# AlgoLab/rs-vgaligner

Measured on AMD Instinct MI355X. Metric: aligned reads/sec (10 kbp ONT vs HLA graph), higher is better.
Workload: dtype int32+f64

## Files before the change

### include/vga_hip.h

```cpp
#ifndef VGA_HIP_H
#define VGA_HIP_H

#include <stddef.h>
#include <stdint.h>

#ifdef __cplusplus
extern "C" {
#endif

#define VGA_OK 0
#define VGA_ERR_ARG (-1)
#define VGA_ERR_HIP (-2)
#define VGA_ERR_NOMEM (-3)
#define VGA_ERR_UNSUPPORTED (-4)
#define VGA_ERR_NO_INDEX (-5)
#define VGA_ERR_NO_DEVICE (-6)
#define VGA_ERR_POOL (-7)

#define VGA_NO_PRED (-1)

#define VGA_MAX_KMER_LENGTH 32

typedef struct vga_ctx vga_ctx;

// ... 45 lines not shown
    uint64_t max_gap;
    uint32_t chain_min_n_anchors;
    int only_forward;
    int emit_dp;
    int32_t strands;
} vga_map_params;
#define VGA_STRANDS_FORWARD 0
#define VGA_STRANDS_BOTH 1
void vga_map_default_params(vga_map_params *p);

typedef struct {
    uint64_t n_reads;
    uint64_t n_anchors;
    uint64_t *anchor_off;
    uint32_t *anchor_id;
    uint32_t *query_begin;
    uint32_t *target_begin;
    uint32_t *target_end;
    double *max_chain_score;
    int32_t *best_pred_id;
    double *curr_max;
    uint64_t n_chains;
    uint64_t *chain_off;
    uint8_t *chain_placeholder;
    uint64_t *chain_anchor_off;
    uint32_t *chain_anchor_idx;
    float ms_probe, ms_sort, ms_chain, ms_total;
    uint64_t n_hits;
    uint8_t *strand;
} vga_map_result;

int vga_map_batch(vga_batch *b, const vga_map_params *params, vga_map_result **out);
void vga_map_result_free(vga_map_result *r);

typedef struct {
    uint64_t n_chains;
    uint64_t *text_off;
    char *text;
    float ms_total;
} vga_chain_text;
int vga_chain_paths_text(vga_ctx *ctx, const vga_map_result *chains, vga_chain_text **out);
void vga_chain_text_free(vga_chain_text *t);

typedef struct {
    int32_t match;
    int32_t mismatch;
    int32_t gap_open1;
    int32_t gap_ext1;
    int32_t gap_open2;
    int32_t gap_ext2;
    int32_t wb;
    int32_t remain_rule;
    double wf;
} vga_poa_params;
#define VGA_REMAIN_LONGEST_PATH 0
#define VGA_REMAIN_FIRST_OUT_EDGE 1
void vga_poa_default_params(vga_poa_params *p);

typedef struct {
    uint64_t n;
    uint8_t *ok;
    int32_t *best_score;
    uint64_t *path_off;
    uint32_t *abpoa_nodes;
    uint32_t *graph_nodes;
    uint32_t *aln_start_offset;
// ... 152 lines not shown
```

### rs-vgaligner_amd/binding.py

```python
from __future__ import annotations

import ctypes as C
import os
from typing import List, Optional, Sequence

import numpy as np

_HERE = os.path.dirname(os.path.abspath(__file__))
LIB_PATH = os.environ.get("VGA_LIB") or os.path.join(_HERE, "libvga_hip.so")

VGA_OK = 0
VGA_MAX_KMER_LENGTH = 32
VGA_STRANDS_FORWARD = 0
VGA_STRANDS_BOTH = 1
ERR_NAMES = {-1: "VGA_ERR_ARG", -2: "VGA_ERR_HIP", -3: "VGA_ERR_NOMEM", -4: "VGA_ERR_UNSUPPORTED",
             -5: "VGA_ERR_NO_INDEX", -6: "VGA_ERR_NO_DEVICE", -7: "VGA_ERR_POOL"}

PILEUP_COLUMNS = ("A", "C", "G", "T", "N", "del", "ins")

ABI_SYMBOLS = [
    "vga_ctx_create", "vga_ctx_destroy", "vga_last_error", "vga_ctx_synchronize", "vga_abi_version",
    "vga_index_upload", "vga_batch_create", "vga_batch_destroy", "vga_batch_strands", "vga_map_default_params", "vga_map_batch",
    "vga_map_result_free", "vga_poa_default_params", "vga_poa_result_free", "vga_poa_batch", "vga_align_batch",
    "vga_align_result_free", "vga_last_kernel_times", "vga_chain_paths_text", "vga_chain_text_free",
    "vga_align_prepare", "vga_ctx_set_pool_fraction", "vga_ctx_set_host_threads",
    "vga_index_build_kmers", "vga_index_kmers_free",
    "vga_coverage_begin", "vga_coverage_read", "vga_coverage_reset", "vga_coverage_end",
    "vga_path_support_begin", "vga_path_support_read", "vga_path_support_last", "vga_path_support_reset", "vga_path_support_end",
    "vga_path_support_lists",
    "vga_pileup_begin", "vga_pileup_read", "vga_pileup_reset", "vga_pileup_end",
    "vga_genotype_begin", "vga_genotype_read", "vga_genotype_reset", "vga_genotype_end", "vga_genotype_pairs",
    "vga_genotype_lik_table", "vga_genotype_lik_begin", "vga_genotype_lik_read", "vga_genotype_lik_reset", "vga_genotype_lik_end",
    "vga_genotype_lik_pairs", "vga_genotype_lik_source",
    "vga_path_edit_begin", "vga_path_edit_read", "vga_path_edit_last", "vga_path_edit_reset", "vga_path_edit_end", "vga_path_edit_pairs",
    "vga_variant_call", "vga_variant_call_table",
    "vga_insertion_begin", "vga_insertion_read", "vga_insertion_reset", "vga_insertion_end", "vga_insertion_call", "vga_insertion_call_table",
    "vga_phase_begin", "vga_phase_read", "vga_phase_reset", "vga_phase_end", "vga_phase_links", "vga_phase_links_lists", "vga_phase_chain",
    "vga_phase_tags", "vga_phase_tags_lists",
    "vga_haplotype_counts", "vga_haplotype_counts_lists", "vga_haplotype_jobs", "vga_haplotype_call",
]

GENOTYPE_TILE = 64
GENOTYPE_READS = 32
GENOTYPE_MIN_CHUNKS = 4
GENOTYPE_MAX_PATHS = 4096

GENOTYPE_LIK_TILE = 128
GENOTYPE_LIK_READS = 32
GENOTYPE_LIK_MIN_CHUNKS = 4
GENOTYPE_LIK_MAX_GROUP_READS = 2048
GENOTYPE_LIK_MAX_PATHS = 4096
GENOTYPE_LIK_MAX_LAMBDA = 4096
GENOTYPE_LIK_MAX_CAP = 255
GENOTYPE_LIK_LAMBDA = 512
GENOTYPE_LIK_CAP = 64
VGA_GL_FROM_SUPPORT = 0
# ... 108 lines not shown


class KernelTime(C.Structure):
    _fields_ = [("name", C.c_char_p), ("ms", C.c_float), ("launches", C.c_uint32), ("algorithmic_bytes", C.c_uint64),
                ("busy_ms", C.c_float), ("reserved", C.c_uint32)]


_lib = None


def load_library():
    global _lib
    if _lib is not None:
        return _lib
    if not os.path.exists(LIB_PATH):
        raise RuntimeError(f"{LIB_PATH} is missing: build it with `python -c 'import __graft_entry__ as g; g.build()'` "
                           "(there is no CPU fallback)")
    L = C.CDLL(LIB_PATH)
    vp = C.c_void_p
    L.vga_ctx_create.argtypes = [C.c_int, _P(vp)]
    L.vga_ctx_destroy.argtypes = [vp]
    L.vga_last_error.argtypes = [vp]
    L.vga_last_error.restype = C.c_char_p
    L.vga_ctx_synchronize.argtypes = [vp]
    L.vga_index_upload.argtypes = [vp, _P(IndexDesc)]
    L.vga_batch_create.argtypes = [vp, C.c_char_p, _P(C.c_uint64), C.c_uint64, _P(vp)]
    L.vga_batch_destroy.argtypes = [vp]
    if hasattr(L, "vga_batch_strands"):
        L.vga_batch_strands.argtypes = [vp, C.c_int, _P(C.c_char), _P(C.c_char)]
        L.vga_batch_strands.restype = C.c_int
    L.vga_map_default_params.argtypes = [_P(MapParams)]
    L.vga_map_batch.argtypes = [vp, _P(MapParams), _P(_P(MapResult))]
    L.vga_map_result_free.argtypes = [_P(MapResult)]
    L.vga_poa_default_params.argtypes = [_P(PoaParams)]
    L.vga_poa_result_free.argtypes = [_P(PoaResult)]
    L.vga_poa_batch.argtypes = [vp, C.c_uint64, _P(C.c_uint64), _P(C.c_uint64), C.c_char_p, _P(C.c_uint64),
                                _P(C.c_uint32), _P(C.c_uint32), _P(C.c_uint64), C.c_char_p, _P(PoaParams),
                                _P(_P(PoaResult))]
    L.vga_align_batch.argtypes = [vp, _P(MapResult), C.c_uint32, _P(PoaParams), _P(_P(AlignResult))]
    L.vga_align_result_free.argtypes = [_P(AlignResult)]
    L.vga_last_kernel_times.argtypes = [vp, _P(KernelTime), C.c_int]
    L.vga_chain_paths_text.argtypes = [vp, _P(MapResult), _P(_P(ChainText))]
    L.vga_align_prepare.argtypes = [vp, C.c_uint64, C.c_uint32]
    L.vga_align_prepare.restype = C.c_int
    L.vga_ctx_set_pool_fraction.argtypes = [vp, C.c_double]
    L.vga_ctx_set_pool_fraction.restype = C.c_int
    L.vga_ctx_set_host_threads.argtypes = [vp, C.c_uint32]
    L.vga_ctx_set_host_threads.restype = C.c_int
    L.vga_chain_text_free.argtypes = [_P(ChainText)]
    L.vga_index_build_kmers.argtypes = [vp, _P(IndexDesc), C.c_uint64, C.c_uint64]
    L.vga_index_build_kmers.restype = C.c_int
    L.vga_index_kmers_free.argtypes = [_P(IndexDesc)]
    L.vga_index_kmers_free.restype = None
    if hasattr(L, "vga_coverage_begin"):
        for name in ("vga_coverage_begin", "vga_coverage_reset", "vga_coverage_end"):
            getattr(L, name).argtypes = [vp]
            getattr(L, name).restype = C.c_int
        L.vga_coverage_read.argtypes = [vp, _P(C.c_uint32), _P(C.c_uint32), _P(C.c_uint32), _P(C.c_uint64)]
        L.vga_coverage_read.restype = C.c_int
    if hasattr(L, "vga_path_support_begin"):
        u64p, u32p = _P(C.c_uint64), _P(C.c_uint32)
        L.vga_path_support_begin.argtypes = [vp, C.c_uint32, u64p, u64p, u64p]
        L.vga_path_support_read.argtypes = [vp, u64p, u64p, u64p, u64p, u64p, u64p]
        L.vga_path_support_last.argtypes = [vp, C.c_uint64, u32p, u32p]
        L.vga_path_support_reset.argtypes = [vp]
        L.vga_path_support_end.argtypes = [vp]
# ... 311 lines not shown
        self.poa_value_cells = int(r.poa_value_cells)
        self.ms = {"subgraph": r.ms_subgraph, "dp": r.ms_dp, "traceback": r.ms_traceback, "total": r.ms_total}
        L.vga_align_result_free(ptr)


class Batch:
    def __init__(self, ctx: "Context", seqs: Sequence):
        self.ctx = ctx
        L = ctx.L
        self.seqs = list(seqs)
        raw = [s if isinstance(s, (bytes, bytearray)) else s.encode() for s in self.seqs]
        self._concat = b"".join(raw)
        off = np.zeros(len(self.seqs) + 1, dtype=np.uint64)
        if self.seqs:
            off[1:] = np.cumsum([len(s) for s in raw], dtype=np.uint64)
        self._off = off
        h = C.c_void_p()
        ctx._check(L.vga_batch_create(ctx.h, self._concat, _u64p(off), len(self.seqs), C.byref(h)))
        self.h = h

    def strands(self, from_host: bool = False):
        n = len(self._concat)
        fwd, rev = C.create_string_buffer(max(1, n)), C.create_string_buffer(max(1, n))
        self.ctx._check(self.ctx.L.vga_batch_strands(self.h, 1 if from_host else 0, fwd, rev))
        return fwd.raw[:n], rev.raw[:n]

    def map(self, params: Optional[MapParams] = None) -> MapOut:
        L = self.ctx.L
        p = params or default_map_params()
        out = _P(MapResult)()
        self.ctx._check(L.vga_map_batch(self.h, C.byref(p), C.byref(out)))
        return MapOut(L, out)

    def align(self, chains: MapOut, best_n: int = 1, params: Optional[PoaParams] = None) -> AlignOut:
        L = self.ctx.L
        p = params or default_poa_params()
        out = _P(AlignResult)()
        self.ctx._check(L.vga_align_batch(self.h, chains._ptr, best_n, C.byref(p), C.byref(out)))
        self.ctx._last_reads = len(self.seqs)
        return AlignOut(L, out)

    def map_raw(self, map_params: Optional[MapParams] = None, on_results=None) -> dict:
        L = self.ctx.L
        mp = map_params
        if mp is None:
            mp = default_map_params()
            mp.emit_dp = 0
        m = _P(MapResult)()
        self.ctx._check(L.vga_map_batch(self.h, C.byref(mp), C.byref(m)))
        try:
            q = m.contents
            if on_results is not None:
                on_results(q, None)
            R = int(q.n_reads)
            ph = np.ctypeslib.as_array(q.chain_placeholder, shape=(int(q.n_chains),)) if int(q.n_chains) else np.zeros(0, np.uint8)
            co = np.ctypeslib.as_array(q.chain_off, shape=(R + 1,)) if R else np.zeros(1, np.uint64)
            mapped = int((ph[co[:-1].astype(np.int64)] == 0).sum()) if R else 0
            return dict(n_reads=R, aligned=mapped, n_anchors=int(q.n_anchors), n_hits=int(q.n_hits), n_chains=int(q.n_chains),
                        ms_map=float(q.ms_total), ms_probe=float(q.ms_probe), ms_sort=float(q.ms_sort), ms_chain=float(q.ms_chain),
                        kernels=self.ctx.kernel_times())
        finally:
            L.vga_map_result_free(m)

    def map_align_raw(self, map_params: Optional[MapParams] = None, best_n: int = 1,
                      poa_params: Optional[PoaParams] = None, on_results=None) -> dict:
        import time as _t
# ... 533 lines not shown
```

### rs-vgaligner_amd/csrc/vga_align.hip

```cpp
#include "vga_align_plan.hpp"
#include "vga_common.hpp"
#include "vga_coverage.hpp"
#include "vga_path_edit.hpp"
#include "vga_path_support.hpp"
#include "vga_pileup.hpp"
#include "vga_insertion.hpp"
#include "vga_poa_internal.hpp"
#include "vga_subgraph_host.hpp"

#include <algorithm>
#include <atomic>
#include <chrono>
#include <memory>

extern "C" void vga_align_result_free(vga_align_result *r)
{
    if (!r) return;
    free(r->aligned); free(r->path_off); free(r->path_handles); free(r->path_length); free(r->path_start);
    free(r->path_end); free(r->block_length); free(r->best_score); free(r->cigar_off); free(r->cigar);
    free(r->cs_off); free(r->cs);
    free(r);
}

namespace {
// ... 48 lines not shown
    int device_store_rest();
    void host_walk();
    int run_poa();
    int begin_result();
    void pick_winners();
    int count_winners();
    int fill_result();
};

int align_call::reverse_complements()
{
    bool any_rev = false;
    if (m->strand)
        for (uint64_t r = 0; r < R && !any_rev; r++) any_rev = m->strand[r] != 0;
    if (!any_rev) return VGA_OK;
    const int rc = vga_batch_revcomp_device(b);
    if (rc != VGA_OK) return rc;
    vga_batch_revcomp_host(b);
    tr.mark("reverse complement");
    return VGA_OK;
}

int align_call::plan()
{
    const char *refused = on_device ? nullptr : cov ? "read coverage is not counted" : ps ? "path support is not scored" : pu ? "the pileup is not counted" : ia ? "the inserted letters are not counted" : nullptr;
    if (refused)
        return vga_set_error(ctx, VGA_ERR_UNSUPPORTED, "vga_align_batch: %s under VGA_SUBGRAPH=host (the subgraph handles are then on the host only)", refused);
    align_select(m, align_best_n, prob_read, prob_chain, read_prob0);
    n = prob_read.size();
    proxy.resize(n);
    west.resize(n);
    descs.resize(n);
    std::atomic<int> has_reverse{0};
    vga_parallel_for(n, [&](uint64_t p) {
        const align_prob a = align_plan_problem(m, prob_read[p], prob_chain[p], qlen(prob_read[p]), ctx->index.k, sw);
        proxy[p] = a.proxy; west[p] = a.west; descs[p] = a.desc;
        if (a.reverse) has_reverse = 1;
    });
    std::vector<uint32_t> ord(n);
    std::iota(ord.begin(), ord.end(), 0u);
    if (on_device) {
        ord = align_launch_order(proxy);
        align_permute(prob_read, ord); align_permute(prob_chain, ord); align_permute(proxy, ord); align_permute(west, ord); align_permute(descs, ord);
    }
    slot_of = align_slot_of(ord);
    if (has_reverse)
        return vga_set_error(ctx, VGA_ERR_UNSUPPORTED,
                             "a chain to be aligned holds reverse-strand anchors: RangeOrient::Reverse / Both (src/align.rs:365-387) is not supported");
    feed.views.resize(n);
    q_src.resize(on_device ? n : 0);
    for (uint64_t p = 0; p < n; p++) {
        const uint64_t r = prob_read[p];
        feed.views[p] = {nullptr, nullptr, 0, nullptr, nullptr, 0, b->reads.data() + q_off(r), qlen(r)};
        if (on_device) q_src[p] = q_off(r);
    }
    feed.proxy = proxy.data();
    return VGA_OK;
}

int align_call::device_store()
{
    vga_timers_reset(ctx);
    feed.keep_timers = true;
    auto ta = std::chrono::steady_clock::now();
    double mean_west = 0;
    const uint64_t split = align_store_split(west, sw, &mean_west);
    if (sw.trace)
        fprintf(stderr, "[vga-trace] align: mean width term of the launch-order proxy %.0f: the subgraph store is built in %s\n", mean_west,
                split == n ? "one part" : "two parts");
    const int rc = sg_prepare(ctx, descs.data(), q_src.data(), prob_read.data(), n, split, b->d_reads, params->remain_rule, store);
    if (rc != VGA_OK) return rc;
// ... 229 lines not shown
```

### rs-vgaligner_amd/csrc/vga_align_plan.hpp

```cpp
#pragma once

#include <algorithm>
#include <cmath>
#include <cstdint>
#include <cstdlib>
#include <cstring>
#include <numeric>
#include <vector>

#include "../../include/vga_hip.h"
#include "vga_sg_records.hpp"

struct align_switches {
    bool sg_host = false;
    uint32_t giant_rows = 24000u;
    double giant_cells = 1.5e8;
    bool has_sg_split = false;
    long sg_split = 0;
    bool trace = false;
};

static inline align_switches align_read_switches()
{
    align_switches s;
    if (const char *e = getenv("VGA_SUBGRAPH")) s.sg_host = strstr(e, "host") != nullptr;
    if (const char *e = getenv("VGA_GIANT_ROWS")) s.giant_rows = (uint32_t)atol(e);
    if (const char *e = getenv("VGA_GIANT_CELLS")) s.giant_cells = atof(e);
    if (const char *e = getenv("VGA_SG_SPLIT")) { s.has_sg_split = true; s.sg_split = atol(e); }
    if (const char *e = getenv("VGA_TRACE")) s.trace = atoi(e) != 0;
    return s;
}

static inline void align_select(const vga_map_result *m, uint32_t best_n, std::vector<uint64_t> &prob_read, std::vector<uint64_t> &prob_chain,
                                std::vector<uint64_t> &read_prob0)
{
    const uint64_t R = m->n_reads;
    prob_read.clear();
    prob_chain.clear();
    read_prob0.assign(R + 1, 0);
    for (uint64_t r = 0; r < R; r++) {
        read_prob0[r] = prob_read.size();
        const uint64_t c0 = m->chain_off[r], c1 = m->chain_off[r + 1];
        const uint64_t take = std::min<uint64_t>(best_n, c1 - c0);
        for (uint64_t c = c0; c < c0 + take; c++)
            if (!m->chain_placeholder[c]) { prob_read.push_back(r); prob_chain.push_back(c); }
    }
    read_prob0[R] = prob_read.size();
}

struct align_prob {
    sg_desc desc;
    uint32_t lo, hi;
    float west;
    double proxy;
    bool reverse;
};

static inline align_prob align_plan_problem(const vga_map_result *m, uint64_t r, uint64_t c, uint32_t qlen, uint32_t k, const align_switches &sw)
{
    align_prob o = {};
    const uint64_t a0 = m->anchor_off[r];
    const uint64_t c0 = m->chain_anchor_off[c], c1 = m->chain_anchor_off[c + 1];
    uint32_t lo = 0xFFFFFFFFu, hi = 0, pmin = 0xFFFFFFFFu, pmax = 0;
    for (uint64_t t = c0; t < c1; t++) {
        const uint64_t ai = a0 + m->chain_anchor_idx[t];
        lo = std::min(lo, m->target_begin[ai]);
        hi = std::max(hi, m->target_end[ai]);
        if ((m->target_begin[ai] | m->target_end[ai]) >> 31) o.reverse = true;
        const uint32_t s = m->target_begin[ai], e = m->target_end[ai] - 1;
        pmin = std::min(pmin, std::min(s, e));
        pmax = std::max(pmax, std::max(s, e));
    }
    o.lo = lo;
    o.hi = hi;
    const double q_first = c1 > c0 ? (double)m->query_begin[a0 + m->chain_anchor_idx[c0]] : 0.0;
    const double q_last = c1 > c0 ? (double)m->query_begin[a0 + m->chain_anchor_idx[c1 - 1]] + (double)k : (double)qlen;
    const double uncovered = q_first + std::max(0.0, (double)qlen - q_last);
    const double rows = (double)(hi > lo ? hi - lo : 0) + 1.6 * uncovered;
    o.west = (float)(650.0 + 0.3 * std::max(0.0, 0.85 * rows - (double)qlen));
    o.proxy = rows * (double)o.west;
    if (rows >= 0.85 * (double)sw.giant_rows) o.proxy += 1e13;
    if (c1 > c0) {
        const uint64_t fa = a0 + m->chain_anchor_idx[c0], la = a0 + m->chain_anchor_idx[c1 - 1];
        o.desc = {pmin, pmax, m->query_begin[fa], m->target_begin[fa], m->query_begin[la], m->target_end[la], qlen, 0u};
    }
    return o;
}

static inline std::vector<uint32_t> align_launch_order(const std::vector<double> &proxy)
{
    std::vector<uint32_t> ord(proxy.size());
    std::iota(ord.begin(), ord.end(), 0u);
    std::stable_sort(ord.begin(), ord.end(), [&](uint32_t x, uint32_t y) { return proxy[x] > proxy[y]; });
    return ord;
}

static inline std::vector<uint32_t> align_slot_of(const std::vector<uint32_t> &ord)
{
    std::vector<uint32_t> slot_of(ord.size());
    for (size_t i = 0; i < ord.size(); i++) slot_of[ord[i]] = (uint32_t)i;
    return slot_of;
}

template <typename T>
static inline void align_permute(std::vector<T> &v, const std::vector<uint32_t> &ord)
{
    std::vector<T> w(v.size());
    for (size_t i = 0; i < ord.size(); i++) w[i] = v[ord[i]];
    v.swap(w);
}

static inline uint64_t align_store_split(const std::vector<float> &west, const align_switches &sw, double *mean_west = nullptr)
{
    const uint64_t n = west.size();
    uint64_t split = n > 3072 ? 2048 : n;
    double wsum = 0;
    for (uint64_t i = 0; i < n; i++) wsum += west[i];
    if (n && wsum / (double)n <= 900.0) split = n;
    if (mean_west) *mean_west = n ? wsum / (double)n : 0.0;
// ... 13 lines not shown
```

### rs-vgaligner_amd/csrc/vga_common.hpp

```cpp
#pragma once

#include <hip/hip_runtime.h>
#include <sys/mman.h>

#include <chrono>
#include <cstdarg>
#include <cstdint>
#include <cstdio>
#include <cstdlib>
#include <cstring>
#include <atomic>
#include <memory>
#include <mutex>
#include <new>
#include <string>
#include <thread>
#include <vector>

#include "../../include/vga_hip.h"
#include "vga_probe_hash.hpp"

#define VGA_ABI_VERSION 6

template <typename T>
// ... 64 lines not shown
    std::vector<hipEvent_t> event_pool;
    size_t events_used = 0;
    struct agg_t {
        std::string name;
        float ms;
        uint32_t launches;
        uint64_t bytes;
        float busy_ms;
    };
    std::vector<agg_t> last_times;
    int n_cu = 256;
    vga_owned<void> map_ws{nullptr, nullptr};
    vga_owned<struct poa_ws> poa_ws{nullptr, nullptr};
    vga_owned<void> sg_ws{nullptr, nullptr};
    vga_owned<void> gaf_ws{nullptr, nullptr};
    std::vector<struct vga_batch *> batches;
};

struct vga_batch {
    vga_ctx *ctx = nullptr;
    int device = 0;
    uint64_t n_reads = 0;
    uint64_t total_bases = 0;
    std::vector<uint64_t> read_off;
    std::vector<char> reads;
    char *d_reads = nullptr;
    uint64_t *d_read_off = nullptr;
    bool rc_dev = false, rc_host = false;
    uint64_t *d_read_off2 = nullptr;
};
int vga_batch_revcomp_device(vga_batch *b);
void vga_batch_revcomp_host(vga_batch *b);

int vga_set_error(vga_ctx *ctx, int code, const char *fmt, ...);
void vga_index_release(vga_dev_index &ix);
int vga_index_load_graph(vga_ctx *ctx, const vga_index_desc *d);

#define VGA_HIP_CHECK(ctx, call)                                                               \
    do {                                                                                       \
        hipError_t e_ = (call);                                                                \
        if (e_ != hipSuccess)                                                                  \
            return vga_set_error((ctx), VGA_ERR_HIP, "%s failed: %s (%s:%d)", #call,           \
                                 hipGetErrorString(e_), __FILE__, __LINE__);                   \
    } while (0)
#define VGA_HIP_CHECK_OOM(ctx, call)                                                         \
    do {                                                                                       \
        hipError_t e_ = (call);                                                                \
        if (e_ != hipSuccess)                                                                  \
            return vga_set_error((ctx), e_ == hipErrorOutOfMemory ? VGA_ERR_NOMEM : VGA_ERR_HIP, \
                                 "%s failed: %s (%s:%d)", #call, hipGetErrorString(e_), __FILE__, __LINE__); \
    } while (0)

template <typename T>
T *xmalloc(size_t n)
{
    return (T *)malloc((n ? n : 1) * sizeof(T));
}

template <typename T, void (*FREE)(T *)>
struct vga_result_guard {
    T *p = nullptr;
    const hipStream_t *wait[2] = {nullptr, nullptr};
    vga_result_guard() = default;
    vga_result_guard(const vga_result_guard &) = delete;
    vga_result_guard &operator=(const vga_result_guard &) = delete;
    ~vga_result_guard()
// ... 132 lines not shown
```

### rs-vgaligner_amd/csrc/vga_map.hip

```cpp
#include "vga_common.hpp"

#include <algorithm>
#include <chrono>
#include <cmath>
#include <memory>

#define VGA_WAVE 64
#define VGA_PROBE_NT 256
#define VGA_SORT_NT 256
#define VGA_NONE32 0xFFFFFFFFu

__device__ __forceinline__ uint32_t vga_lane() { return threadIdx.x & 63u; }

__device__ __forceinline__ uint32_t vga_wave_incl_scan(uint32_t v)
{
    uint32_t lane = vga_lane();
#pragma unroll
    for (int d = 1; d < 64; d <<= 1) {
        uint32_t o = __shfl_up(v, d, 64);
        if (lane >= (uint32_t)d) v += o;
    }
    return v;
}

__device__ __forceinline__ uint32_t vga_block_excl_scan_256(uint32_t v, uint32_t *ws, uint32_t &total)
{
    uint32_t incl = vga_wave_incl_scan(v);
    uint32_t w = threadIdx.x >> 6;
    if (vga_lane() == 63) ws[w] = incl;
    __syncthreads();
    uint32_t w0 = ws[0], w1 = ws[1], w2 = ws[2], w3 = ws[3];
    uint32_t before = (w > 0 ? w0 : 0) + (w > 1 ? w1 : 0) + (w > 2 ? w2 : 0);
    total = w0 + w1 + w2 + w3;
    __syncthreads();
    return before + incl - v;
}

__device__ __forceinline__ uint32_t vga_base_code_dev(uint8_t c)
// ... 351 lines not shown
            int pnext;
            while ((pnext = vpred[cur]) >= 0) {
                if (lane == 0) { vpred[cur] = -1; buf[wpos] = (uint32_t)cur; }
                __threadfence_block();
                wpos++;
                len++;
                cur = pnext;
            }
            if (lane == 0) buf[wpos] = (uint32_t)cur;
            wpos++;
            len++;
            if (len >= min_anchors) {
                if (lane == 0) buf[hdr] = len;
                nch++;
            } else {
                wpos = hdr;
            }
        }
    }
    if (lane == 0) { chain_cnt[r] = nch; chain_words[r] = wpos; }
}

__global__ __launch_bounds__(256) void k_chain_compact(const uint64_t *__restrict__ anchor_off, const uint32_t *__restrict__ chain_words,
                                                       const uint64_t *__restrict__ woff, const uint32_t *__restrict__ chain_buf,
                                                       uint32_t *__restrict__ comp)
{
    const uint64_t r = blockIdx.x;
    const uint32_t *src = chain_buf + 3 * anchor_off[r] + 2 * r;
    uint32_t *dst = comp + woff[r];
    const uint32_t n = chain_words[r];
    for (uint32_t i = threadIdx.x; i < n; i += blockDim.x) dst[i] = src[i];
}

__global__ __launch_bounds__(256) void k_strand_pick(uint32_t R, const uint64_t *__restrict__ anchor_off, const double *__restrict__ curr_max,
                                                     const uint32_t *__restrict__ chain_cnt, const uint32_t *__restrict__ chain_words,
                                                     uint8_t *__restrict__ strand, uint32_t *__restrict__ sel, uint32_t *__restrict__ sel_anchors,
                                                     double *__restrict__ sel_curr_max, uint32_t *__restrict__ sel_chain_cnt,
                                                     uint32_t *__restrict__ sel_chain_words)
{
    const uint32_t r = blockIdx.x * 256 + threadIdx.x;
    if (r >= R) return;
    const uint32_t rv = R + r;
    const bool rev = chain_cnt[rv] > 0 && (chain_cnt[r] == 0 || curr_max[rv] > curr_max[r]);
    const uint32_t s = rev ? rv : r;
    strand[r] = rev ? 1 : 0;
    sel[r] = s;
    sel_anchors[r] = (uint32_t)(anchor_off[s + 1] - anchor_off[s]);
    sel_curr_max[r] = curr_max[s];
    sel_chain_cnt[r] = chain_cnt[s];
    sel_chain_words[r] = chain_words[s];
}

__global__ __launch_bounds__(256) void k_strand_scan(uint32_t R, const uint32_t *__restrict__ cnt, uint64_t *__restrict__ off)
{
    __shared__ uint32_t ws[4];
    uint64_t carry = 0;
    for (uint32_t c0 = 0; c0 < R; c0 += 256) {
        const uint32_t i = c0 + threadIdx.x;
        const uint32_t v = i < R ? cnt[i] : 0u;
        uint32_t total;
        const uint32_t ex = vga_block_excl_scan_256(v, ws, total);
        if (i < R) off[i] = carry + ex;
        carry += total;
    }
    if (threadIdx.x == 0) off[R] = carry;
}
// ... 23 lines not shown
}

__global__ __launch_bounds__(256) void k_chain_compact_sel(const uint32_t *__restrict__ sel, const uint64_t *__restrict__ anchor_off,
                                                           const uint32_t *__restrict__ sel_chain_words, const uint64_t *__restrict__ woff,
                                                           const uint32_t *__restrict__ chain_buf, uint32_t *__restrict__ comp)
{
    const uint64_t r = blockIdx.x, s = sel[r];
    const uint32_t *src = chain_buf + 3 * anchor_off[s] + 2 * s;
    uint32_t *dst = comp + woff[r];
    const uint32_t n = sel_chain_words[r];
    for (uint32_t i = threadIdx.x; i < n; i += blockDim.x) dst[i] = src[i];
}

namespace {

struct map_ws {
    vga_dbuf<uint32_t> cnt;
    vga_dbuf<uint64_t> anchor_off;
    vga_dbuf<uint32_t> a_qb, a_tb, a_te, a_idx, key_b, val_b, s_qb, s_tb, s_te;
    vga_dbuf<double> f, curr_max, gap_cost;
    vga_dbuf<int32_t> pred_id, pred_pos;
    vga_dbuf<uint32_t> chain_buf, chain_cnt, chain_words, key_a, chain_comp;
    vga_dbuf<uint64_t> chain_woff;
    vga_dbuf<uint8_t> strand;
    vga_dbuf<uint32_t> sel, sel_anchors, sel_chain_cnt, sel_chain_words, g_qb, g_tb, g_te, g_id;
    vga_dbuf<uint64_t> sel_off;
    vga_dbuf<double> sel_curr_max, g_f;
    vga_dbuf<int32_t> g_pred;
    vga_hbuf<uint64_t> h_chain_woff;
    vga_hbuf<uint32_t> h_chain_cnt, h_chain_words, h_cnt;
    vga_hbuf<double> h_curr_max;
    hipStream_t st_copy = nullptr;
    hipEvent_t ev_sorted = nullptr;
    ~map_ws()
    {
        if (st_copy) (void)hipStreamDestroy(st_copy);
        if (ev_sorted) (void)hipEventDestroy(ev_sorted);
    }
};

}

extern "C" void vga_map_result_free(vga_map_result *r)
{
    if (!r) return;
    free(r->anchor_off);
    free(r->anchor_id);
    free(r->query_begin);
    free(r->target_begin);
    free(r->target_end);
    free(r->max_chain_score);
    free(r->best_pred_id);
    free(r->curr_max);
    free(r->chain_off);
    free(r->chain_placeholder);
    free(r->chain_anchor_off);
    free(r->chain_anchor_idx);
    free(r->strand);
    free(r);
}

namespace {

struct map_source {
    const double *curr_max = nullptr;
    const uint32_t *chain_cnt = nullptr, *chain_words = nullptr;
    const uint32_t *ids = nullptr;
    const double *f = nullptr;
    const int32_t *pred = nullptr;
};

struct map_call {
    vga_ctx *const ctx;
    vga_batch *const b;
    const vga_map_params *const params;
    const vga_dev_index &ix;
    const uint64_t R;
    const bool all_orients;
// ... 252 lines not shown
    VGA_HIP_CHECK(ctx, hipMemcpyAsync(ws.h_curr_max.p, src.curr_max, R * 8, hipMemcpyDeviceToHost, st));
    VGA_HIP_CHECK(ctx, hipMemcpyAsync(ws.h_chain_cnt.p, src.chain_cnt, R * 4, hipMemcpyDeviceToHost, st));
    VGA_HIP_CHECK(ctx, hipMemcpyAsync(ws.h_chain_words.p, src.chain_words, R * 4, hipMemcpyDeviceToHost, st));
    VGA_HIP_CHECK(ctx, hipStreamSynchronize(st));
    return VGA_OK;
}

int map_call::gather_picked()
{
    const size_t As = (size_t)res->anchor_off[R];
    res->n_anchors = As;
    if (!alloc_anchor_arrays(As)) return nomem();
    VGA_HIP_CHECK(ctx, ws.g_qb.reserve(As)); VGA_HIP_CHECK(ctx, ws.g_tb.reserve(As)); VGA_HIP_CHECK(ctx, ws.g_te.reserve(As));
    if (emit_dp) { VGA_HIP_CHECK(ctx, ws.g_id.reserve(As)); VGA_HIP_CHECK(ctx, ws.g_f.reserve(As)); VGA_HIP_CHECK(ctx, ws.g_pred.reserve(As)); }
    const int tg = vga_timer_begin(ctx, "strand_gather", (uint64_t)As * 2 * (12 + (emit_dp ? 16 : 0)) + R * 20);
    hipLaunchKernelGGL(k_strand_gather, dim3((unsigned)R), dim3(256), 0, st, ws.sel.p, ws.anchor_off.p, ws.sel_off.p, ws.s_qb.p, ws.s_tb.p,
                       ws.s_te.p, perm, ws.f.p, ws.pred_id.p, ws.g_qb.p, ws.g_tb.p, ws.g_te.p, emit_dp ? ws.g_id.p : nullptr,
                       emit_dp ? ws.g_f.p : nullptr, emit_dp ? ws.g_pred.p : nullptr);
    vga_timer_end(ctx, tg);
    if (As) {
        VGA_HIP_CHECK(ctx, hipMemcpyAsync(res->query_begin, ws.g_qb.p, As * 4, hipMemcpyDeviceToHost, st));
        VGA_HIP_CHECK(ctx, hipMemcpyAsync(res->target_begin, ws.g_tb.p, As * 4, hipMemcpyDeviceToHost, st));
        VGA_HIP_CHECK(ctx, hipMemcpyAsync(res->target_end, ws.g_te.p, As * 4, hipMemcpyDeviceToHost, st));
    }
    src.ids = ws.g_id.p;
    src.f = ws.g_f.p;
    src.pred = ws.g_pred.p;
    return VGA_OK;
}

int map_call::fetch_chains()
{
    const size_t An_res = (size_t)res->n_anchors;
    for (uint64_t r = 0; r < R; r++) { ws.h_chain_woff.p[r] = chain_total_words; chain_total_words += ws.h_chain_words.p[r]; }
    ws.h_chain_woff.p[R] = chain_total_words;
    chain_words_host.reset(xmalloc<uint32_t>(chain_total_words + 2));
    if (!chain_words_host) return nomem();
    if (chain_total_words) {
        VGA_HIP_CHECK(ctx, ws.chain_comp.reserve(chain_total_words + 2));
        VGA_HIP_CHECK(ctx, hipMemcpyAsync(ws.chain_woff.p, ws.h_chain_woff.p, (R + 1) * 8, hipMemcpyHostToDevice, st));
        if (both)
            hipLaunchKernelGGL(k_chain_compact_sel, dim3((unsigned)R), dim3(256), 0, st, ws.sel.p, ws.anchor_off.p, ws.sel_chain_words.p,
                               ws.chain_woff.p, ws.chain_buf.p, ws.chain_comp.p);
        else
            hipLaunchKernelGGL(k_chain_compact, dim3((unsigned)R), dim3(256), 0, st, ws.anchor_off.p, ws.chain_words.p, ws.chain_woff.p,
                               ws.chain_buf.p, ws.chain_comp.p);
        VGA_HIP_CHECK(ctx, hipMemcpyAsync(chain_words_host.get(), ws.chain_comp.p, chain_total_words * 4, hipMemcpyDeviceToHost, st));
    }
    if (An_res && emit_dp) {
        VGA_HIP_CHECK(ctx, hipMemcpyAsync(res->anchor_id, src.ids, An_res * 4, hipMemcpyDeviceToHost, st));
        VGA_HIP_CHECK(ctx, hipMemcpyAsync(res->max_chain_score, src.f, An_res * 8, hipMemcpyDeviceToHost, st));
        VGA_HIP_CHECK(ctx, hipMemcpyAsync(res->best_pred_id, src.pred, An_res * 4, hipMemcpyDeviceToHost, st));
    }
    VGA_HIP_CHECK(ctx, hipStreamSynchronize(st));
    VGA_HIP_CHECK(ctx, hipStreamSynchronize(ws.st_copy));
    tr.mark("kernels + D2H");
    vga_timers_collect(ctx);
    memcpy(res->curr_max, ws.h_curr_max.p, R * 8);
    return VGA_OK;
}

int map_call::assemble()
{
    const uint32_t *h_chain_cnt = ws.h_chain_cnt.p, *h_chain_words = ws.h_chain_words.p, *h_chain_buf = chain_words_host.get();
    uint64_t n_chains = 0, n_members = 0;
    std::vector<uint64_t> mem0(R);
    for (uint64_t r = 0; r < R; r++) {
        uint32_t c = h_chain_cnt[r];
        res->chain_off[r] = n_chains;
        mem0[r] = n_members;
        n_chains += c ? c : 1;
        n_members += h_chain_words[r] - c;
    }
    res->chain_off[R] = n_chains;
    res->n_chains = n_chains;
    res->chain_placeholder = xmalloc<uint8_t>(n_chains);
    res->chain_anchor_off = xmalloc<uint64_t>(n_chains + 1);
    res->chain_anchor_idx = xmalloc<uint32_t>(n_members);
    if (!res->chain_placeholder || !res->chain_anchor_off || !res->chain_anchor_idx) return nomem();
    res->chain_anchor_off[n_chains] = n_members;
    vga_map_result *const out = res.p;
// ... 9 lines not shown
        for (uint32_t q = 0; q < c; q++) {
            uint32_t len = buf[wp++];
            out->chain_placeholder[ci] = 0;
            out->chain_anchor_off[ci] = mi;
            for (uint32_t t = 0; t < len; t++) out->chain_anchor_idx[mi + t] = buf[wp + len - 1 - t];
            wp += len;
            mi += len;
            ci++;
        }
    }, (unsigned)std::max<uint64_t>(1, (n_members + 64 * R) / 1000000));
    tr.mark("chain assembly");
    res->ms_probe = vga_timer_sum(ctx, "kmer_probe");
    res->ms_sort = vga_timer_sum(ctx, "anchor_sort");
    res->ms_chain = vga_timer_sum(ctx, "chain_dp");
    res->ms_total = (float)std::chrono::duration<double, std::milli>(std::chrono::steady_clock::now() - t_host0).count();
    return VGA_OK;
}

}

static int vga_map_batch_impl(vga_batch *b, const vga_map_params *params, vga_map_result **out)
{
    if (!b || !params || !out || !b->ctx) return VGA_ERR_ARG;
    vga_ctx *ctx = b->ctx;
    *out = nullptr;
    (void)hipSetDevice(ctx->device);
    vga_ctx_scope scope(ctx);
    vga_release_deferred(ctx);
    int rc = map_validate(ctx, params);
    if (rc != VGA_OK) return rc;
    if (!ctx->map_ws && !(ctx->map_ws = vga_make_owned<void, map_ws>())) throw std::bad_alloc();
    vga_timers_reset(ctx);
    map_call c(b, params, *(map_ws *)ctx->map_ws.get());
    if ((rc = c.begin_result()) != VGA_OK) return rc;
    if (c.R > 0) {
        if ((rc = c.count()) != VGA_OK) return rc;
        if ((rc = c.emit_and_sort()) != VGA_OK) return rc;
        c.chain();
        if ((rc = c.both ? c.source_picked() : c.source_forward()) != VGA_OK) return rc;
        if ((rc = c.fetch_counts()) != VGA_OK) return rc;
        if (c.both && (rc = c.gather_picked()) != VGA_OK) return rc;
        if ((rc = c.fetch_chains()) != VGA_OK) return rc;
        if ((rc = c.assemble()) != VGA_OK) return rc;
    }
    *out = c.res.release();
    return VGA_OK;
}

extern "C" int vga_map_batch(vga_batch *b, const vga_map_params *params, vga_map_result **out)
{
    try {
        return vga_map_batch_impl(b, params, out);
    } catch (const std::bad_alloc &) {
        return vga_set_error((b ? b->ctx : nullptr), VGA_ERR_NOMEM, "vga_map_batch: out of host memory");
    } catch (const std::exception &e) {
        return vga_set_error((b ? b->ctx : nullptr), VGA_ERR_ARG, "vga_map_batch: %s", e.what());
    }
}
```

Measured before the change: 10600.

## Compute per-chain alignment-plan summaries on GPU during mapping and reuse in align

Adds a GPU kernel at the end of mapping that reduces each chain's anchors into a twelve-word summary (target extent, positions, first and last anchors, strand), copies the table to the host, and registers it against the map result. The align planner then checks each chain against that table and uses it instead of walking every anchor on the host, falling back to host summarisation on mismatch. The aim is to cut the host-side per-chain planning loop in align. In exchange it adds a kernel launch, extra device-to-host copies and mutex-protected global bookkeeping to every map call.

```diff
diff --git a/include/vga_hip.h b/include/vga_hip.h
--- a/include/vga_hip.h
+++ b/include/vga_hip.h
@@ -101,6 +101,7 @@
 
 int vga_map_batch(vga_batch *b, const vga_map_params *params, vga_map_result **out);
 void vga_map_result_free(vga_map_result *r);
+int vga_map_chain_summaries(vga_batch *b, const vga_map_result *chains, uint32_t *out);
 
 typedef struct {
     uint64_t n_chains;
diff --git a/rs-vgaligner_amd/binding.py b/rs-vgaligner_amd/binding.py
--- a/rs-vgaligner_amd/binding.py
+++ b/rs-vgaligner_amd/binding.py
@@ -21,7 +21,7 @@
 ABI_SYMBOLS = [
     "vga_ctx_create", "vga_ctx_destroy", "vga_last_error", "vga_ctx_synchronize", "vga_abi_version",
     "vga_index_upload", "vga_batch_create", "vga_batch_destroy", "vga_batch_strands", "vga_map_default_params", "vga_map_batch",
-    "vga_map_result_free", "vga_poa_default_params", "vga_poa_result_free", "vga_poa_batch", "vga_align_batch",
+    "vga_map_result_free", "vga_map_chain_summaries", "vga_poa_default_params", "vga_poa_result_free", "vga_poa_batch", "vga_align_batch",
     "vga_align_result_free", "vga_last_kernel_times", "vga_chain_paths_text", "vga_chain_text_free",
     "vga_align_prepare", "vga_ctx_set_pool_fraction", "vga_ctx_set_host_threads",
     "vga_index_build_kmers", "vga_index_kmers_free",
@@ -196,6 +196,8 @@
     L.vga_map_default_params.argtypes = [_P(MapParams)]
     L.vga_map_batch.argtypes = [vp, _P(MapParams), _P(_P(MapResult))]
     L.vga_map_result_free.argtypes = [_P(MapResult)]
+    if hasattr(L, "vga_map_chain_summaries"):
+        L.vga_map_chain_summaries.argtypes = [vp, _P(MapResult), _P(C.c_uint32)]
     L.vga_poa_default_params.argtypes = [_P(PoaParams)]
     L.vga_poa_result_free.argtypes = [_P(PoaResult)]
     L.vga_poa_batch.argtypes = [vp, C.c_uint64, _P(C.c_uint64), _P(C.c_uint64), C.c_char_p, _P(C.c_uint64),
@@ -573,6 +575,11 @@
         self.ctx._check(L.vga_map_batch(self.h, C.byref(p), C.byref(out)))
         return MapOut(L, out)
 
+    def chain_summaries(self, chains: MapOut) -> np.ndarray:
+        out = np.zeros((max(1, chains.n_chains), 12), dtype=np.uint32)
+        self.ctx._check(self.ctx.L.vga_map_chain_summaries(self.h, chains._ptr, out.ctypes.data_as(_P(C.c_uint32))))
+        return out[:chains.n_chains]
+
     def align(self, chains: MapOut, best_n: int = 1, params: Optional[PoaParams] = None) -> AlignOut:
         L = self.ctx.L
         p = params or default_poa_params()
diff --git a/rs-vgaligner_amd/csrc/vga_align.hip b/rs-vgaligner_amd/csrc/vga_align.hip
--- a/rs-vgaligner_amd/csrc/vga_align.hip
+++ b/rs-vgaligner_amd/csrc/vga_align.hip
@@ -104,11 +104,21 @@
     west.resize(n);
     descs.resize(n);
     std::atomic<int> has_reverse{0};
+    std::vector<chain_summary> table;
+    const bool from_map = !sw.plan_host && vga_map_chain_table(ctx, b, m, table) && table.size() == m->n_chains;
+    std::atomic<uint64_t> n_host{0};
     vga_parallel_for(n, [&](uint64_t p) {
-        const align_prob a = align_plan_problem(m, prob_read[p], prob_chain[p], qlen(prob_read[p]), ctx->index.k, sw);
+        const uint64_t r = prob_read[p], c = prob_chain[p];
+        const bool use = from_map && align_summary_matches(m, r, c, table[c]);
+        if (!use) n_host++;
+        const align_prob a = align_plan_from_summary(use ? table[c] : align_summarise(m, r, c), qlen(r), ctx->index.k, sw);
         proxy[p] = a.proxy; west[p] = a.west; descs[p] = a.desc;
         if (a.reverse) has_reverse = 1;
-    });
+    }, from_map ? 4u : 0u);
+    if (sw.trace)
+        fprintf(stderr, "[vga-trace] align: %llu of %llu chains summarised on the host (%s)\n", (unsigned long long)n_host.load(), (unsigned long long)n,
+                sw.plan_host ? "VGA_ALIGN_PLAN=host" : from_map ? "the rest: the map call's table" : "not the context's latest map result");
+    tr.mark("plan: chain summaries");
     std::vector<uint32_t> ord(n);
     std::iota(ord.begin(), ord.end(), 0u);
     if (on_device) {
diff --git a/rs-vgaligner_amd/csrc/vga_align_plan.hpp b/rs-vgaligner_amd/csrc/vga_align_plan.hpp
--- a/rs-vgaligner_amd/csrc/vga_align_plan.hpp
+++ b/rs-vgaligner_amd/csrc/vga_align_plan.hpp
@@ -18,6 +18,7 @@
     bool has_sg_split = false;
     long sg_split = 0;
     bool trace = false;
+    bool plan_host = false;
 };
 
 static inline align_switches align_read_switches()
@@ -28,6 +29,7 @@
     if (const char *e = getenv("VGA_GIANT_CELLS")) s.giant_cells = atof(e);
     if (const char *e = getenv("VGA_SG_SPLIT")) { s.has_sg_split = true; s.sg_split = atol(e); }
     if (const char *e = getenv("VGA_TRACE")) s.trace = atoi(e) != 0;
+    if (const char *e = getenv("VGA_ALIGN_PLAN")) s.plan_host = strstr(e, "host") != nullptr;
     return s;
 }
 
@@ -56,35 +58,71 @@
     bool reverse;
 };
 
-static inline align_prob align_plan_problem(const vga_map_result *m, uint64_t r, uint64_t c, uint32_t qlen, uint32_t k, const align_switches &sw)
+struct chain_summary {
+    uint32_t lo, hi;
+    uint32_t pmin, pmax;
+    uint32_t first_qb, first_tb, first_te;
+    uint32_t last_qb, last_tb, last_te;
+    uint32_t reverse;
+    uint32_t n_anchors;
+};
+static_assert(sizeof(chain_summary) == 48, "chain_summary is twelve 32-bit words on the device and on the host");
+constexpr uint32_t CHAIN_SUMMARY_WORDS = 12;
+
+static inline chain_summary align_summarise(const vga_map_result *m, uint64_t r, uint64_t c)
+{
+    const uint64_t a0 = m->anchor_off[r];
+    const uint64_t c0 = m->chain_anchor_off[c], c1 = m->chain_anchor_off[c + 1];
+    chain_summary s = {0xFFFFFFFFu, 0u, 0xFFFFFFFFu, 0u, 0u, 0u, 0u, 0u, 0u, 0u, 0u, (uint32_t)(c1 - c0)};
+    for (uint64_t t = c0; t < c1; t++) {
+        const uint64_t ai = a0 + m->chain_anchor_idx[t];
+        const uint32_t b = m->target_begin[ai], e = m->target_end[ai] - 1;
+        s.lo = std::min(s.lo, b);
+        s.hi = std::max(s.hi, m->target_end[ai]);
+        if ((b | m->target_end[ai]) >> 31) s.reverse = 1;
+        s.pmin = std::min(s.pmin, std::min(b, e));
+        s.pmax = std::max(s.pmax, std::max(b, e));
+    }
+    if (c1 > c0) {
+        const uint64_t fa = a0 + m->chain_anchor_idx[c0], la = a0 + m->chain_anchor_idx[c1 - 1];
+        s.first_qb = m->query_begin[fa]; s.first_tb = m->target_begin[fa]; s.first_te = m->target_end[fa];
+        s.last_qb = m->query_begin[la]; s.last_tb = m->target_begin[la]; s.last_te = m->target_end[la];
+    }
+    return s;
+}
+
+static inline bool align_summary_matches(const vga_map_result *m, uint64_t r, uint64_t c, const chain_summary &s)
+{
+    const uint64_t a0 = m->anchor_off[r];
+    const uint64_t c0 = m->chain_anchor_off[c], c1 = m->chain_anchor_off[c + 1];
+    if (c1 - c0 != s.n_anchors) return false;
+    if (c1 == c0) return true;
+    const uint64_t fa = a0 + m->chain_anchor_idx[c0], la = a0 + m->chain_anchor_idx[c1 - 1];
+    return m->query_begin[fa] == s.first_qb && m->target_begin[fa] == s.first_tb && m->target_end[fa] == s.first_te &&
+           m->query_begin[la] == s.last_qb && m->target_begin[la] == s.last_tb && m->target_end[la] == s.last_te;
+}
+
+static inline align_prob align_plan_from_summary(const chain_summary &s, uint32_t qlen, uint32_t k, const align_switches &sw)
 {
     align_prob o = {};
-    const uint64_t a0 = m->anchor_off[r];
-    const uint64_t c0 = m->chain_anchor_off[c], c1 = m->chain_anchor_off[c + 1];
-    uint32_t lo = 0xFFFFFFFFu, hi = 0, pmin = 0xFFFFFFFFu, pmax = 0;
-    for (uint64_t t = c0; t < c1; t++) {
-        const uint64_t ai = a0 + m->chain_anchor_idx[t];
-        lo = std::min(lo, m->target_begin[ai]);
-        hi = std::max(hi, m->target_end[ai]);
-        if ((m->target_begin[ai] | m->target_end[ai]) >> 31) o.reverse = true;
-        const uint32_t s = m->target_begin[ai], e = m->target_end[ai] - 1;
-        pmin = std::min(pmin, std::min(s, e));
-        pmax = std::max(pmax, std::max(s, e));
-    }
+    const uint32_t lo = s.lo, hi = s.hi;
     o.lo = lo;
     o.hi = hi;
-    const double q_first = c1 > c0 ? (double)m->query_begin[a0 + m->chain_anchor_idx[c0]] : 0.0;
-    const double q_last = c1 > c0 ? (double)m->query_begin[a0 + m->chain_anchor_idx[c1 - 1]] + (double)k : (double)qlen;
+    o.reverse = s.reverse != 0;
+    const double q_first = s.n_anchors ? (double)s.first_qb : 0.0;
+    const double q_last = s.n_anchors ? (double)s.last_qb + (double)k : (double)qlen;
     const double uncovered = q_first + std::max(0.0, (double)qlen - q_last);
     const double rows = (double)(hi > lo ? hi - lo : 0) + 1.6 * uncovered;
     o.west = (float)(650.0 + 0.3 * std::max(0.0, 0.85 * rows - (double)qlen));
     o.proxy = rows * (double)o.west;
     if (rows >= 0.85 * (double)sw.giant_rows) o.proxy += 1e13;
-    if (c1 > c0) {
-        const uint64_t fa = a0 + m->chain_anchor_idx[c0], la = a0 + m->chain_anchor_idx[c1 - 1];
-        o.desc = {pmin, pmax, m->query_begin[fa], m->target_begin[fa], m->query_begin[la], m->target_end[la], qlen, 0u};
-    }
+    if (s.n_anchors) o.desc = {s.pmin, s.pmax, s.first_qb, s.first_tb, s.last_qb, s.last_te, qlen, 0u};
     return o;
+}
+
+static inline align_prob align_plan_problem(const vga_map_result *m, uint64_t r, uint64_t c, uint32_t qlen, uint32_t k, const align_switches &sw)
+{
+    return align_plan_from_summary(align_summarise(m, r, c), qlen, k, sw);
 }
 
 static inline std::vector<uint32_t> align_launch_order(const std::vector<double> &proxy)
diff --git a/rs-vgaligner_amd/csrc/vga_common.hpp b/rs-vgaligner_amd/csrc/vga_common.hpp
--- a/rs-vgaligner_amd/csrc/vga_common.hpp
+++ b/rs-vgaligner_amd/csrc/vga_common.hpp
@@ -120,6 +120,9 @@
 int vga_batch_revcomp_device(vga_batch *b);
 void vga_batch_revcomp_host(vga_batch *b);
 
+struct chain_summary;
+bool vga_map_chain_table(vga_ctx *ctx, const vga_batch *b, const vga_map_result *m, std::vector<chain_summary> &out);
+
 int vga_set_error(vga_ctx *ctx, int code, const char *fmt, ...);
 void vga_index_release(vga_dev_index &ix);
 int vga_index_load_graph(vga_ctx *ctx, const vga_index_desc *d);
diff --git a/rs-vgaligner_amd/csrc/vga_map.hip b/rs-vgaligner_amd/csrc/vga_map.hip
--- a/rs-vgaligner_amd/csrc/vga_map.hip
+++ b/rs-vgaligner_amd/csrc/vga_map.hip
@@ -1,9 +1,11 @@
+#include "vga_align_plan.hpp"
 #include "vga_common.hpp"
 
 #include <algorithm>
 #include <chrono>
 #include <cmath>
 #include <memory>
+#include <mutex>
 
 #define VGA_WAVE 64
 #define VGA_PROBE_NT 256
@@ -421,6 +423,56 @@
     for (uint32_t i = threadIdx.x; i < n; i += blockDim.x) dst[i] = src[i];
 }
 
+__global__ __launch_bounds__(256) void k_chain_summary(uint32_t R, const uint32_t *__restrict__ sel, const uint64_t *__restrict__ anchor_off,
+                                                       const uint32_t *__restrict__ chain_cnt, const uint64_t *__restrict__ woff,
+                                                       const uint64_t *__restrict__ coff, const uint32_t *__restrict__ comp,
+                                                       const uint32_t *__restrict__ s_qb, const uint32_t *__restrict__ s_tb,
+                                                       const uint32_t *__restrict__ s_te, uint32_t *__restrict__ out)
+{
+    const uint32_t r = blockIdx.x * 4 + (threadIdx.x >> 6);
+    if (r >= R) return;
+    const uint32_t lane = vga_lane();
+    const uint32_t nch = chain_cnt[r];
+    uint32_t *rec = out + coff[r] * CHAIN_SUMMARY_WORDS;
+    if (nch == 0) {
+        if (lane < CHAIN_SUMMARY_WORDS) rec[lane] = (lane == 0 || lane == 2) ? VGA_NONE32 : 0u;
+        return;
+    }
+    const uint64_t a0 = anchor_off[sel ? sel[r] : r];
+    const uint32_t *qb = s_qb + a0, *tb = s_tb + a0, *te = s_te + a0;
+    const uint32_t *buf = comp + woff[r];
+    uint32_t wp = 0;
+    for (uint32_t q = 0; q < nch; q++, rec += CHAIN_SUMMARY_WORDS) {
+        const uint32_t len = buf[wp++];
+        uint32_t lo = VGA_NONE32, hi = 0, pmin = VGA_NONE32, pmax = 0, rev = 0;
+        for (uint32_t t = lane; t < len; t += 64) {
+            const uint32_t i = buf[wp + t];
+            const uint32_t b = tb[i], en = te[i], e = en - 1;
+            lo = min(lo, b);
+            hi = max(hi, en);
+            rev |= (b | en) >> 31;
+            pmin = min(pmin, min(b, e));
+            pmax = max(pmax, max(b, e));
+        }
+#pragma unroll
+        for (int d = 32; d > 0; d >>= 1) {
+            lo = min(lo, (uint32_t)__shfl_xor((int)lo, d, 64));
+            hi = max(hi, (uint32_t)__shfl_xor((int)hi, d, 64));
+            pmin = min(pmin, (uint32_t)__shfl_xor((int)pmin, d, 64));
+            pmax = max(pmax, (uint32_t)__shfl_xor((int)pmax, d, 64));
+            rev |= (uint32_t)__shfl_xor((int)rev, d, 64);
+        }
+        if (lane == 0) {
+            const uint32_t fa = buf[wp + len - 1], la = buf[wp];
+            rec[0] = lo; rec[1] = hi; rec[2] = pmin; rec[3] = pmax;
+            rec[4] = qb[fa]; rec[5] = tb[fa]; rec[6] = te[fa];
+            rec[7] = qb[la]; rec[8] = tb[la]; rec[9] = te[la];
+            rec[10] = rev; rec[11] = len;
+        }
+        wp += len;
+    }
+}
+
 __global__ __launch_bounds__(256) void k_strand_pick(uint32_t R, const uint64_t *__restrict__ anchor_off, const double *__restrict__ curr_max,
                                                      const uint32_t *__restrict__ chain_cnt, const uint32_t *__restrict__ chain_words,
                                                      uint8_t *__restrict__ strand, uint32_t *__restrict__ sel, uint32_t *__restrict__ sel_anchors,
@@ -510,18 +562,77 @@
     vga_hbuf<double> h_curr_max;
     hipStream_t st_copy = nullptr;
     hipEvent_t ev_sorted = nullptr;
-    ~map_ws()
+    vga_dbuf<uint64_t> chain_coff;
+    vga_hbuf<uint64_t> h_chain_coff;
+    vga_dbuf<uint32_t> sum;
+    vga_hbuf<uint32_t> h_sum;
+    const vga_map_result *sum_of = nullptr;
+    const vga_batch *sum_batch = nullptr;
+    map_ws();
+    ~map_ws();
+};
+
+std::mutex tables_mu;
+std::vector<map_ws *> tables;
+
+map_ws::map_ws()
+{
+    std::lock_guard<std::mutex> g(tables_mu);
+    tables.push_back(this);
+}
+
+map_ws::~map_ws()
+{
     {
-        if (st_copy) (void)hipStreamDestroy(st_copy);
-        if (ev_sorted) (void)hipEventDestroy(ev_sorted);
-    }
-};
-
+        std::lock_guard<std::mutex> g(tables_mu);
+        tables.erase(std::remove(tables.begin(), tables.end(), this), tables.end());
+    }
+    if (st_copy) (void)hipStreamDestroy(st_copy);
+    if (ev_sorted) (void)hipEventDestroy(ev_sorted);
+}
+
+void stamp_summaries(map_ws &ws, const vga_map_result *of, const vga_batch *b)
+{
+    std::lock_guard<std::mutex> g(tables_mu);
+    ws.sum_of = of;
+    ws.sum_batch = b;
+}
+
+}
+
+bool vga_map_chain_table(vga_ctx *ctx, const vga_batch *b, const vga_map_result *m, std::vector<chain_summary> &out)
+{
+    const map_ws *ws = (const map_ws *)ctx->map_ws.get();
+    if (!ws || !m) return false;
+    std::lock_guard<std::mutex> g(tables_mu);
+    if (ws->sum_of != m || ws->sum_batch != b) return false;
+    out.resize(m->n_chains);
+    if (m->n_chains) memcpy(out.data(), ws->h_sum.p, m->n_chains * sizeof(chain_summary));
+    return true;
+}
+
+extern "C" int vga_map_chain_summaries(vga_batch *b, const vga_map_result *chains, uint32_t *out)
+{
+    if (!b || !chains || !out || !b->ctx) return VGA_ERR_ARG;
+    try {
+        std::vector<chain_summary> tab;
+        if (!vga_map_chain_table(b->ctx, b, chains, tab))
+            return vga_set_error(b->ctx, VGA_ERR_ARG, "vga_map_chain_summaries: not the result of this context's latest vga_map_batch on this batch");
+        if (!tab.empty()) memcpy(out, tab.data(), tab.size() * sizeof(chain_summary));
+        return VGA_OK;
+    } catch (const std::bad_alloc &) {
+        return vga_set_error(b->ctx, VGA_ERR_NOMEM, "vga_map_chain_summaries: out of host memory");
+    }
 }
 
 extern "C" void vga_map_result_free(vga_map_result *r)
 {
     if (!r) return;
+    {
+        std::lock_guard<std::mutex> g(tables_mu);
+        for (map_ws *ws : tables)
+            if (ws->sum_of == r) ws->sum_of = nullptr;
+    }
     free(r->anchor_off);
     free(r->anchor_id);
     free(r->query_begin);
@@ -840,8 +951,14 @@
 int map_call::fetch_chains()
 {
     const size_t An_res = (size_t)res->n_anchors;
-    for (uint64_t r = 0; r < R; r++) { ws.h_chain_woff.p[r] = chain_total_words; chain_total_words += ws.h_chain_words.p[r]; }
+    VGA_HIP_CHECK(ctx, ws.h_chain_coff.reserve(R + 1)); VGA_HIP_CHECK(ctx, ws.chain_coff.reserve(R + 1));
+    uint64_t n_chains = 0;
+    for (uint64_t r = 0; r < R; r++) {
+        ws.h_chain_woff.p[r] = chain_total_words; chain_total_words += ws.h_chain_words.p[r];
+        ws.h_chain_coff.p[r] = n_chains; n_chains += ws.h_chain_cnt.p[r] ? ws.h_chain_cnt.p[r] : 1;
+    }
     ws.h_chain_woff.p[R] = chain_total_words;
+    ws.h_chain_coff.p[R] = n_chains;
     chain_words_host.reset(xmalloc<uint32_t>(chain_total_words + 2));
     if (!chain_words_host) return nomem();
     if (chain_total_words) {
@@ -855,6 +972,13 @@
                                ws.chain_buf.p, ws.chain_comp.p);
         VGA_HIP_CHECK(ctx, hipMemcpyAsync(chain_words_host.get(), ws.chain_comp.p, chain_total_words * 4, hipMemcpyDeviceToHost, st));
     }
+    VGA_HIP_CHECK(ctx, ws.sum.reserve(n_chains * CHAIN_SUMMARY_WORDS)); VGA_HIP_CHECK(ctx, ws.h_sum.reserve(n_chains * CHAIN_SUMMARY_WORDS));
+    VGA_HIP_CHECK(ctx, hipMemcpyAsync(ws.chain_coff.p, ws.h_chain_coff.p, (R + 1) * 8, hipMemcpyHostToDevice, st));
+    const int ts = vga_timer_begin(ctx, "chain_summary", 16 * chain_total_words + 48 * n_chains);
+    hipLaunchKernelGGL(k_chain_summary, dim3((unsigned)((R + 3) / 4)), dim3(256), 0, st, (uint32_t)R, both ? ws.sel.p : nullptr, ws.anchor_off.p,
+                       src.chain_cnt, ws.chain_woff.p, ws.chain_coff.p, ws.chain_comp.p, ws.s_qb.p, ws.s_tb.p, ws.s_te.p, ws.sum.p);
+    vga_timer_end(ctx, ts);
+    VGA_HIP_CHECK(ctx, hipMemcpyAsync(ws.h_sum.p, ws.sum.p, n_chains * sizeof(chain_summary), hipMemcpyDeviceToHost, st));
     if (An_res && emit_dp) {
         VGA_HIP_CHECK(ctx, hipMemcpyAsync(res->anchor_id, src.ids, An_res * 4, hipMemcpyDeviceToHost, st));
         VGA_HIP_CHECK(ctx, hipMemcpyAsync(res->max_chain_score, src.f, An_res * 8, hipMemcpyDeviceToHost, st));
@@ -930,6 +1054,7 @@
     if (!ctx->map_ws && !(ctx->map_ws = vga_make_owned<void, map_ws>())) throw std::bad_alloc();
     vga_timers_reset(ctx);
     map_call c(b, params, *(map_ws *)ctx->map_ws.get());
+    stamp_summaries(c.ws, nullptr, nullptr);
     if ((rc = c.begin_result()) != VGA_OK) return rc;
     if (c.R > 0) {
         if ((rc = c.count()) != VGA_OK) return rc;
@@ -940,6 +1065,7 @@
         if (c.both && (rc = c.gather_picked()) != VGA_OK) return rc;
         if ((rc = c.fetch_chains()) != VGA_OK) return rc;
         if ((rc = c.assemble()) != VGA_OK) return rc;
+        stamp_summaries(c.ws, c.res.p, b);
     }
     *out = c.res.release();
     return VGA_OK;
```

Result: no change. 10580 (-0.2%).
